# nka77/DAHiTra

Hardware: AMD Instinct MI355X
Metric: image-pairs/s (256x256) train step, 1/2/4/8 MI355X + CPU ref (higher is better)
Workload: dtype bf16; 1 GPU; LEVIR-CD 256x256 synthetic pairs, base_transformer_pos_s4, bf16, batch 32 per GPU (global 32), fwd+focal+bwd+allreduce+AdamW; net_G=base_transformer_pos_s4, global_batch=32, img_size=256, parallelism=dp1, hip_graph=True, step_form=one graph (AdamW inside), attn_dtype=bf16

## Files before the change

### dahitra_amd/csrc/head_fwd.hip

```cpp
#include "common.h"

namespace {

constexpr int HF_KP = 18;
constexpr int HF_SLOTS = 4;

typedef __attribute__((ext_vector_type(4))) unsigned u32x4;
typedef __attribute__((ext_vector_type(8))) _Float16 hf_f16x8;
constexpr int HF_GPW = 5;

template <typename T, bool INBN>
__global__ __launch_bounds__(256) void head_fwd_kernel(const T* __restrict__ x, const float* __restrict__ w_oihw,
                                                       const float* __restrict__ bias, int NC, const float* __restrict__ in_scale,
                                                       const float* __restrict__ in_shift, int in_groups, float* __restrict__ out,
                                                       int N, int H, int W, int rpb) {
    extern __shared__ __attribute__((aligned(16))) float smem[];
    const int RS = (W + 2) * HF_KP;
    const int tid = threadIdx.x, lane = tid & 63, wv = tid >> 6, pl = lane & 15, g = lane >> 4;
    const int bpi = (H + rpb - 1) / rpb, n = blockIdx.x / bpi, r0 = (blockIdx.x - n * bpi) * rpb, r1 = min(r0 + rpb, H);
    constexpr bool F32 = sizeof(T) == 4;
    constexpr int PL = F32 ? 2 : 1, PXB = 32 * (int)sizeof(T);
    uint4 a0[PL], a1[PL];
    {
        float v0[8], v1[8];
        const int tap = pl >> 1, co = pl & 1;
#pragma unroll
        for (int e = 0; e < 8; ++e) {
            const int ci = 8 * g + e;
            v0[e] = co < NC ? w_oihw[((size_t)co * 32 + ci) * 9 + tap] : 0.f;
            v1[e] = (pl < 2 && pl < NC) ? w_oihw[((size_t)pl * 32 + ci) * 9 + 8] : 0.f;
            if constexpr (F32) { v0[e] *= F32H3_WSCALE; v1[e] *= F32H3_WSCALE; }
        }
        if constexpr (F32) { split_f16_planes(v0, a0); split_f16_planes(v1, a1); }
        else { a0[0] = pack16<bf16>(v0); a1[0] = pack16<bf16>(v1); }
    }
    auto mma = [](const uint4& a, const uint4& b, f32x4 c) {
        if constexpr (F32) return __builtin_amdgcn_mfma_f32_16x16x32_f16(__builtin_bit_cast(hf_f16x8, a), __builtin_bit_cast(hf_f16x8, b), c, 0, 0, 0);
        else return __builtin_amdgcn_mfma_f32_16x16x32_bf16(__builtin_bit_cast(s16x8, a), __builtin_bit_cast(s16x8, b), c, 0, 0, 0);
    };
// ... 67 lines not shown
                *reinterpret_cast<float2*>(p + 4 * g + 2) = make_float2(d0[2], d0[3]);
                if (g == 0) *reinterpret_cast<float2*>(p + 16) = make_float2(d1[0], d1[1]);
            }
        }
    };
    const float b0 = bias ? bias[0] : 0.f, b1 = (bias && NC > 1) ? bias[1] : 0.f;
    auto out_row = [&](int y) {
        const float* s0 = smem + ((y - 1) & (HF_SLOTS - 1)) * RS;
        const float* s1 = smem + (y & (HF_SLOTS - 1)) * RS;
        const float* s2 = smem + ((y + 1) & (HF_SLOTS - 1)) * RS;
        for (int xx = tid; xx < W; xx += 256) {
            float acc0 = b0, acc1 = b1;
#pragma unroll
            for (int kh = 0; kh < 3; ++kh) {
                const float* s = kh == 0 ? s0 : (kh == 1 ? s1 : s2);
#pragma unroll
                for (int kw = 0; kw < 3; ++kw) {
                    const float2 v = *reinterpret_cast<const float2*>(s + (xx + kw) * HF_KP + (kh * 3 + kw) * 2);
                    acc0 += v.x; acc1 += v.y;
                }
            }
            out[(((long)n * NC) * H + y) * W + xx] = acc0;
            if (NC > 1) out[(((long)n * NC + 1) * H + y) * W + xx] = acc1;
        }
    };
    RowRegs qa, qb;
    request(r0 - 1, qa);
    request(r0, qb);
    p_row(r0 - 1, qa);
    request(r0 + 1, qa);
    p_row(r0, qb);
    for (int y = r0; y < r1; y += 2) {
        request(y + 2, qb);
        p_row(y + 1, qa);
        __syncthreads();
        out_row(y);
        if (y + 1 >= r1) break;
        request(y + 3, qa);
        p_row(y + 2, qb);
        __syncthreads();
        out_row(y + 1);
    }
}

}

extern "C" int dh_head_fwd_supported(int NC, int W) { return NC >= 1 && NC <= 2 && (long)HF_SLOTS * (W + 2) * HF_KP * 4 <= 80 * 1024; }
extern "C" int dh_head_fwd(int dtype, const void* x, const float* w_oihw, const float* bias, int NC, const float* in_scale,
                           const float* in_shift, int in_groups, float* logits_nchw, int N, int H, int W, void* stream) {
    DH_REQUIRE(x && w_oihw && logits_nchw && N > 0 && H > 0 && W > 0, "head_fwd: bad arguments");
    DH_REQUIRE(dh_head_fwd_supported(NC, W), "head_fwd: n_class=%d W=%d is not this kernel's shape (dh_head_fwd_supported)", NC, W);
    DH_REQUIRE((long)N * H * W * 128 < (1L << 31), "head_fwd: %d x %d x %d pixels x 128 bytes do not fit a 2 GiB buffer descriptor", N, H, W);
    if (in_scale) DH_REQUIRE(in_shift && in_groups > 0 && N % in_groups == 0, "head_fwd: BatchNorm-on-load needs in_shift and N %% in_groups == 0");
    int rpb = H;
    while (rpb > 8 && (long)N * ((H + rpb / 2 - 1) / (rpb / 2)) <= 512) rpb /= 2;
    const int grid = N * ((H + rpb - 1) / rpb);
    const size_t lds = (size_t)HF_SLOTS * (W + 2) * HF_KP * 4;
    hipStream_t st = reinterpret_cast<hipStream_t>(stream);
    static bool attr_done = false;
    if (!attr_done) {
        DH_REQUIRE(hipFuncSetAttribute(reinterpret_cast<const void*>(head_fwd_kernel<bf16, true>), hipFuncAttributeMaxDynamicSharedMemorySize, 80 * 1024) == hipSuccess &&
                   hipFuncSetAttribute(reinterpret_cast<const void*>(head_fwd_kernel<bf16, false>), hipFuncAttributeMaxDynamicSharedMemorySize, 80 * 1024) == hipSuccess &&
                   hipFuncSetAttribute(reinterpret_cast<const void*>(head_fwd_kernel<float, true>), hipFuncAttributeMaxDynamicSharedMemorySize, 80 * 1024) == hipSuccess &&
                   hipFuncSetAttribute(reinterpret_cast<const void*>(head_fwd_kernel<float, false>), hipFuncAttributeMaxDynamicSharedMemorySize, 80 * 1024) == hipSuccess,
                   "head_fwd: 80 KiB of dynamic LDS refused");
        attr_done = true;
    }
#define HF_LAUNCH(T, BN) hipLaunchKernelGGL((head_fwd_kernel<T, BN>), dim3(grid), dim3(256), lds, st, (const T*)x, w_oihw, bias, NC, in_scale, \
                                            in_shift, BN ? in_groups : 1, logits_nchw, N, H, W, rpb)
    if (dtype == DH_DTYPE_BF16) { if (in_scale) HF_LAUNCH(bf16, true); else HF_LAUNCH(bf16, false); }
    else { if (in_scale) HF_LAUNCH(float, true); else HF_LAUNCH(float, false); }
#undef HF_LAUNCH
    DH_CHECK_LAUNCH("head_fwd");
    return 0;
}
```

### dahitra_amd/csrc/loss_optim.hip

```cpp
#include "common.h"

namespace {

constexpr int MAXC = 8;

template <int CT>
__global__ __launch_bounds__(256) void focal_kernel(const float* __restrict__ logits, const long long* __restrict__ target,
                                                    int B, int Crt, long HW, float alpha, float gscale,
                                                    float* __restrict__ dlogits, float* __restrict__ partial) {
    __shared__ float red[256];
    const int C = CT > 0 ? CT : Crt;
    constexpr int NC = CT > 0 ? CT : MAXC;
    const long total = (long)B * HW;
    float lsum = 0.f;
    const long stride = (long)gridDim.x * blockDim.x;
    const long i0 = (long)blockIdx.x * blockDim.x + threadIdx.x;
    long b = i0 / HW, p = i0 - b * HW;
    const long db = stride / HW, dp = stride - db * HW;
    for (long i = i0; i < total; i += stride) {
        float z[NC], pr[NC], lp[NC];
        float m = -INFINITY;
#pragma unroll
        for (int c = 0; c < NC; ++c)
            if (c < C) { z[c] = logits[(b * C + c) * HW + p]; m = fmaxf(m, z[c]); }
        float s = 0.f;
#pragma unroll
        for (int c = 0; c < NC; ++c)
            if (c < C) { pr[c] = expf(z[c] - m); s += pr[c]; }
        const float ls = logf(s), inv = 1.f / s;
        const int t = (int)target[i];
        float loss = 0.f, gsum = 0.f, gp[NC];
#pragma unroll
        for (int c = 0; c < NC; ++c)
            if (c < C) {
                pr[c] *= inv;
                lp[c] = z[c] - m - ls;
                const float oh = (c == t ? 1.f : 0.f) + 1e-6f;
                const float om = 1.f - pr[c];
                loss += oh * (-alpha * om * om * lp[c]);
                gp[c] = oh * (-alpha) * (-2.f * om * pr[c] * lp[c] + om * om);
                gsum += gp[c];
            }
        lsum += loss;
        if (dlogits) {
#pragma unroll
            for (int c = 0; c < NC; ++c)
                if (c < C) dlogits[(b * C + c) * HW + p] = gscale * (gp[c] - pr[c] * gsum);
        }
        b += db; p += dp;
        if (p >= HW) { p -= HW; ++b; }
    }
    red[threadIdx.x] = lsum;
    __syncthreads();
    for (int o = 128; o > 0; o >>= 1) {
        if (threadIdx.x < o) red[threadIdx.x] += red[threadIdx.x + o];
        __syncthreads();
    }
    if (threadIdx.x == 0) partial[blockIdx.x] = red[0];
}

__global__ __launch_bounds__(256) void ce_partial_kernel(const float* __restrict__ logits, const long long* __restrict__ target,
                                                         int B, int C, long HW, int ignore, double* __restrict__ partial) {
    __shared__ double sh[16];
    double ls = 0.0, cnt = 0.0;
    const long total = (long)B * HW;
    for (long i = (long)blockIdx.x * blockDim.x + threadIdx.x; i < total; i += (long)gridDim.x * blockDim.x) {
        const int t = (int)target[i];
        if (t == ignore) continue;
        const long b = i / HW, p = i % HW;
        float m = -INFINITY;
// ... 352 lines not shown
```

### dahitra_amd/engine.py

```python
import os
import sys
import types

import torch

from . import ops
from .netspec import (ATTN_SCALE, BIT_DIM_HEAD, BIT_HEADS, BN_EPS, BN_MOMENTUM, DIM, LN_EPS, UNET_LEVELS,
                      get_config, is_active, state_spec)

RELU, GELU, NONE = ops.ACT_RELU, ops.ACT_GELU, ops.ACT_NONE



def _drain(gen):
    try:
        while True:
            next(gen)
    except StopIteration as e:
        return e.value


class Packed:
    __slots__ = ("fwd", "dgrad", "fwd_frag", "dgrad_frag")

    def __init__(self, fwd, dgrad, fwd_frag=None, dgrad_frag=None):
        self.fwd, self.dgrad, self.fwd_frag, self.dgrad_frag = fwd, dgrad, fwd_frag, dgrad_frag


class Gated:
    __slots__ = ("g", "partial")

    def __init__(self, g, partial):
        self.g, self.partial = g, partial


class HeadGrad:
    __slots__ = ("dl", "w", "ncls", "gw", "gb")

    def __init__(self, dl, w, ncls, gw, gb):
        self.dl, self.w, self.ncls, self.gw, self.gb = dl, w, ncls, gw, gb


class CoarseRes:
    __slots__ = ("t",)

    def __init__(self, t):
        self.t = t


class MaskedRes:
    __slots__ = ("t", "bits")

    def __init__(self, t, bits):
        self.t, self.bits = t, bits


class Engine:
    def __init__(self, net_G, dtype=torch.float32, use_tr=True, attn_fp8=False, mma_x3=False):
        self.net_G = net_G
        self.mma_x3 = bool(mma_x3) and dtype == torch.float32
        self.mma_fwd = int(os.environ.get("DAHITRA_X3_FWD", "3")) if self.mma_x3 else 0
        self.mma_bwd = int(os.environ.get("DAHITRA_X3_BWD", "1")) if self.mma_x3 else 0
        self._x3_checked = False
        self.attn_fp8 = bool(attn_fp8) or os.environ.get("DAHITRA_ATTN_FP8", "0") == "1"
        self.cfg = get_config(net_G)
        self.dtype = dtype
        self.use_tr = use_tr
        self.fused_decoder = os.environ.get("DAHITRA_NO_FUSED_DECODER", "0") != "1"
        self.fused_encoder = os.environ.get("DAHITRA_NO_FUSED_ENCODER", "0") != "1"
        self.fused_bn_bwd = os.environ.get("DAHITRA_BN_FUSION", "0") == "1"
        self.coarse_shortcut = os.environ.get("DAHITRA_NO_COARSE_SHORTCUT", "0") != "1"
        self.lazy_bn = os.environ.get("DAHITRA_NO_LAZY_BN", "0") != "1"
        self.phase_conv_pred = os.environ.get("DAHITRA_NO_PHASE_CONV", "0") != "1"
        self.phase_s2_dgrad = os.environ.get("DAHITRA_NO_PHASE_S2", "0") != "1"
        self.phase_up_conv = os.environ.get("DAHITRA_NO_PHASE_UPCONV", "0") != "1"
        self.split_cat = os.environ.get("DAHITRA_NO_SPLIT_CAT", "0") != "1"
        self.direct_stem = os.environ.get("DAHITRA_NO_DIRECT_STEM", "0") != "1"
        self.fused_stem_bwd = os.environ.get("DAHITRA_NO_FUSED_STEM_BWD", "0") != "1"
        self.fused_head_out = os.environ.get("DAHITRA_NO_FUSED_HEAD", "0") != "1"
        self.defer_dec_finalize = os.environ.get("DAHITRA_NO_DEFER_DEC_FINALIZE", "0") != "1"
        self.fuse_dec_stack = os.environ.get("DAHITRA_NO_DEC_STACK", "0") != "1"
        self.level_streams = os.environ.get("DAHITRA_LEVEL_STREAMS", "0") == "1"
        self._lstreams = []
        self.gated_head_dgrad = os.environ.get("DAHITRA_GATED_HEAD", "0") == "1"
        self.fused_head_bn = os.environ.get("DAHITRA_NO_FUSED_HEAD_BN", "0") != "1"
        self.fused_up4_bwd = os.environ.get("DAHITRA_NO_FUSED_UP4_BWD", "0") != "1"
        self.fused_up4_fwd = os.environ.get("DAHITRA_FUSED_UP4_FWD", "0") == "1"
        self.use_side = os.environ.get("DAHITRA_SIDE_STREAM", "0") == "1"
        self.block_copies = os.environ.get("DAHITRA_BLOCK_COPIES", "0") == "1"
        self.pack_side = os.environ.get("DAHITRA_PACK_SIDE", "0") == "1"
        self._pack_stream = None
        self.side = None
        self._deferred_wgrad = None
        self.shapes = {k: s for k, s, _ in state_spec(net_G)}
        self.p = {}
        self.g = {}
        self.pk = {}
        self.wstack = {}
        self.training = False
        self.need_grad = False
        self._bwd = None
        self._plans = {}
        self._wgrad_plan = None

    def bind(self, params, grads):
        self.p, self.g = params, grads
        self._plans = {}

# ... 753 lines not shown
    def run_deferred_wgrad(self):
        d, self._deferred_wgrad = self._deferred_wgrad, None
        if d is None:
            return
        x, dy, wkey, ks, stride, pad, dilation = d
        with self.side.fork(x.y if isinstance(x, ops.BnInput) else (x.a if isinstance(x, ops.Up4Input) else x), dy):
            ops.conv2d_wgrad(x, dy, self.g[wkey], ks, stride, pad, accumulate=True, use_tr=self.use_tr, dilation=dilation)

    def _side_join(self):
        if self.side is not None:
            self.run_deferred_wgrad()
            self.side.join()

    def backward_second(self):
        ops.set_f32_mma_mode(self.mma_bwd)
        second, state = self._split_state
        self._split_state = None
        try:
            second(state)
            self._wgrad_plan.run()
        finally:
            self._wgrad_plan.__exit__(*sys.exc_info())

    def _head_out(self, h, wkey, bkey):
        ncls = self.shapes[wkey][0]
        ck = ops.chunk_channels(self.dtype)
        if self.pk[wkey].fwd.shape[-2] == 16 and self.fused_head_out:
            out = ops.conv3x3_head(h, self.pk[wkey].fwd, ncls, self.p[bkey], w_oihw=self.p[wkey])
        else:
            out = ops.nhwc_to_nchw(ops.conv2d(h, self.pk[wkey].fwd, ncls, 3, 1, 1, bias=self.p[bkey]))
        if not self.need_grad:
            return out, None

        small = 8 if (self.dtype == torch.bfloat16 or ncls > 4) else 4
        direct = h.shape[-1] == 32 and ncls <= small

        def bwd(dl_nchw, next_gate=None, head_bn=None, relu_out=None):
            if direct and next_gate is None:
                fuse = self.fused_head_bn and ncls <= 8 and self.g[wkey].is_contiguous() and \
                    (self.dtype == torch.bfloat16 or (self.dtype == torch.float32 and ops.get_f32_mma_mode() != 0))
                if head_bn is not None and fuse:
                    return HeadGrad(ops.head_dlogits_pack(dl_nchw, self.dtype), self.p[wkey], ncls, self.g[wkey], self.g[bkey])
                if relu_out is not None and fuse and relu_out is h:
                    return ops.head_relu_bwd(ops.head_dlogits_pack(dl_nchw, self.dtype), self.p[wkey], ncls, h, self.g[wkey],
                                             self.g[bkey])
                dl = ops.nchw_to_nhwc(dl_nchw, self.dtype, cpad=small)
                ops.conv2d_wgrad(h, dl, self.g[wkey], 3, 1, 1, accumulate=True, use_tr=self.use_tr, cout_real=ncls)
                tmp = torch.empty(small, dtype=torch.float32, device=h.device)
                ops.colsum(dl.view(-1, small), tmp)
                ops.reduce_rows(tmp, 1, ncls, self.g[bkey], accumulate=True)
                if head_bn is not None and self.gated_head_dgrad and self.dtype == torch.bfloat16 and ncls <= 2:
                    return Gated(*ops.head_dgrad3x3_bn(dl, self.p[wkey], ncls, *head_bn))
                return ops.head_dgrad3x3(dl, self.p[wkey], ncls, relu_out=relu_out)
            dl = ops.nchw_to_nhwc(dl_nchw, self.dtype, cpad=ck)
            ops.conv2d_wgrad(h, dl, self.g[wkey], 3, 1, 1, accumulate=True, use_tr=self.use_tr, cout_real=ncls)
            tmp = torch.empty(ck, dtype=torch.float32, device=h.device)
            ops.colsum(dl.view(-1, ck), tmp)
            ops.reduce_rows(tmp, 1, ncls, self.g[bkey], accumulate=True)
            dh = self.conv_dgrad(dl, wkey, 3, 1, 1, h.shape, gate=next_gate)
            return ops.act_bwd(dh, relu_out, RELU) if relu_out is not None else dh
# ... 16 lines not shown
        phased = self.phase_conv_pred and l3.shape[-1] % 64 == 0
        if phased:
            feat, b_pred = self.conv_pred_phase(l3)
        else:
            up = ops.upsample2(l3)
            feat, b_pred = self.conv_act(up, "conv_pred.weight", "conv_pred.bias", 3, 1, NONE)
        _, fh, fw, _ = feat.shape
        hw = fh * fw
        wa = self.p["conv_a.weight"]
        tok_cat, tsaved = ops.tokenizer_fwd(feat, wa, self.p["pos_embedding"], B, L)
        tok2d, b_enc = self.encoder(tok_cat.view(B * 2 * L, DIM), "transformer", cfg["enc_depth"], BIT_HEADS,
                                    BIT_DIM_HEAD, B, 2 * L)
        dtok = torch.zeros_like(tok2d) if self.need_grad else None
        dec, b_dec = self.decoder(feat.view(S2 * hw, DIM), S2, tok2d, 2 * L * DIM, L * DIM, B, dtok,
                                  "transformer_decoder", cfg["dec_depth"], BIT_HEADS, cfg["dec_dim_head"], L)
        dec4 = dec.view(S2, fh, fw, DIM)
        k0 = "classifier.0.weight"
        if self.fused_up4_fwd and self.dtype == torch.bfloat16 and DIM == 32 and tuple(self.shapes[k0][:2]) == (32, 32) and \
                tuple(self.pk[k0].fwd.shape) == (9, 32, 32):
            upd = ops.Up4Input(dec4[:B].contiguous(), dec4[B:].contiguous())
        else:
            upd = ops.absdiff_upsample4(dec4[:B], dec4[B:])
        h, b_c0 = self.conv_bn(upd, k0, "classifier.1", 3, 1, 1, 1, True, lazy=True, side_wgrad=True)
        logits, b_out = self._head_out(h, "classifier.3.weight", "classifier.3.bias")
        if not self.need_grad:
            return logits, None

        def bwd_first(dl):
            dh = b_out(dl, next_gate=b_c0.gate, head_bn=getattr(b_c0, "bn", None))
            fuse = self.fused_up4_bwd and self.dtype == torch.bfloat16 and fh % 2 == 0 and fw % 4 == 0 and \
                self.pk["classifier.0.weight"].dgrad.dim() == 3 and self.pk["classifier.0.weight"].dgrad.shape[1] == 32
            if fuse:
                dec_g = torch.empty_like(dec4)
                b_c0(dh, through_up4=(dec4[:B], dec4[B:], dec_g[:B], dec_g[B:]))
            else:
                dupd, _ = b_c0(dh)
                dec_g = torch.empty_like(dec4)
                ops.absdiff_upsample4_bwd_into(dec4[:B], dec4[B:], dupd, dec_g[:B], dec_g[B:])
            dfeat = b_dec(dec_g.view(S2 * hw, DIM))
            if self.side is not None:
                self.run_deferred_wgrad()
            dtok_cat = b_enc(dtok)
            dfeat4 = dfeat.view(S2, fh, fw, DIM)
            ops.tokenizer_bwd(feat, wa, tsaved, dtok_cat, dfeat4, self.g["conv_a.weight"], self.g["pos_embedding"],
                              B, L, accumulate=True)
            dl3 = b_pred(dfeat4) if phased else ops.upsample2_bwd(b_pred(dfeat4))
            return b_l3(dl3, next_gate=b_l2.gate)
# ... 167 lines not shown
        s4, b_l1 = self.res_layer(p4, 1, 1, 2)
        s8, b_l2 = self.res_layer(s4, 2, 2, 2)
        p16, arg16 = ops.maxpool(s8, want_arg=True)
        s16, b_l3 = self.res_layer(p16, 3, 1, 2)
        level = self._xbd_level if self.cfg["kind"] == "xbd" else self._level
        if self.need_grad:
            self._zpool = [torch.zeros(3 * 3 * B * self.cfg["token_len"] * DIM, dtype=torch.float32, device=s4.device), 0]
        ew = self.cfg["kind"] != "xbd"
        (o5, b5), (t4, b4), (t3, b3) = self._run_staged([level(5, s16, B), level(4, s8, B), level(3, s4, B)], ew=ew)
        self._zpool = None
        o5u = ops.upsample2(o5)
        o4, bu4 = self._up_conv(4, ops.add(t4, o5u))
        o3, bu3 = self._up_conv(3, ops.add(t3, o4))
        _, h2, w2, c2 = s2.shape
        k20 = "conv_layer2_0.0.weight"
        split2 = self.split_cat and self.training and self.pk[k20].fwd_frag is not None and \
            (not self.need_grad or self.pk[k20].dgrad_frag is not None) and \
            ops.conv3x3_split_supported(B, h2, w2, 2 * c2, self.shapes[k20][0], self.dtype)
        cat2 = ops.SplitCat(s2) if split2 else ops.SplitCat(s2).materialize()
        y, b20 = self.conv_bn(cat2, k20, "conv_layer2_0.1", 3, 1, 1, 1, True, lazy=True)
        y2 = ops.conv2d(y, self.pk["conv_layer2_0.3.weight"].fwd, 32, 3, 1, 1, bias=self.p["conv_layer2_0.3.bias"],
                        residual=o3)
        o2, bu2 = self._up_conv(2, y2)
        logits, b_out = self._head_out(o2, "classifier.weight", "classifier.bias")
        if not self.need_grad:
            return logits, None

        def bwd_first(dl):
            do2 = b_out(dl, relu_out=o2)
            dy2 = bu2(do2, masked=True)
            ops.conv2d_wgrad(y, dy2, self.g["conv_layer2_0.3.weight"], 3, 1, 1, accumulate=True, use_tr=self.use_tr)
            ops.colsum(dy2.view(-1, 32), self.g["conv_layer2_0.3.bias"], accumulate=True)
            dy = self.conv_dgrad(dy2, "conv_layer2_0.3.weight", 3, 1, 1, y.shape, gate=b20.gate)
            dcat2, _ = b20(dy)
            if split2:
                ds2 = dcat2
            else:
                ds2 = ops.split_halves(dcat2)
            dsum3 = bu3(dy2)
            dsum4 = bu4(dsum3)
            ds4, ds8, ds16 = self._run_staged([b3(dsum3), b4(dsum4), b5(ops.upsample2_bwd(dsum4))], ew=ew)
            return ds16, ds8, ds4, ds2

        def bwd_second(state):
            ds16, ds8, ds4, ds2 = state
            dp16 = b_l3(ds16)
            ds8 = ops.add(ds8, ops.maxpool_bwd(arg16, dp16, s8.shape))
# ... 12 lines not shown
```

### dahitra_amd/graph.py

```python
import os

import torch
import torch.distributed as dist

from . import ops, parallel
from .models import losses


class GraphedTrainStep:
    CHECK_EVERY = 64

    def __init__(self, net, opt, a, b, lab, warmup=3, confusion=None):
        if not getattr(opt, "capturable", False):
            raise ValueError("GraphedTrainStep needs dahitra_amd.optim.AdamW(..., capturable=True)")
        self.net, self.opt = net, opt
        self.confusion = confusion
        self.world = dist.get_world_size() if dist.is_initialized() else 1
        self.exchange = parallel.exchange_enabled()
        self.split_off = None
        self.persist_bn_launches = None
        self._set_inputs(a, b, lab)
        net._ensure_arena(a.device)
        flat0 = net._arena.flat.clone()
        bufs0 = [t.clone() for t in net.buffers()]
# ... 59 lines not shown
        loss.backward()
        self._count(self.logits)
        if include_opt:
            self.opt.step()
        return loss.detach()

    def _body(self, include_opt):
        if type(self)._eager_body is not GraphedTrainStep._eager_body or os.environ.get("DAHITRA_GRAPH_AUTOGRAD") == "1":
            return self._eager_body(include_opt)
        net = self.net
        logits = self._forward_split()
        bwd = net._engine.take_backward()
        self.logits = logits
        loss, dl = self._loss_and_grad(logits)
        self._count(logits)
        net._arena.grad.zero_()
        net._engine.backward(dl, bwd)
        net._bind_grad_views()
        if include_opt:
            self.opt.step()
        return loss

    def _forward_split(self):
        return self.net._run_forward(self.a, self.b, need_grad=True)

    def _loss_and_grad(self, logits):
        tgt = self.lab[:, 0] if self.lab.dim() == logits.dim() else self.lab
        return ops.focal_loss(logits, tgt.to(torch.int64).contiguous(), want_grad=True)

    def _count(self, logits):
        if self.confusion is not None:
            tgt = self.lab[:, 0] if self.lab.dim() == logits.dim() else self.lab
            ops.confusion_matrix(logits, tgt.to(torch.int64).contiguous(), self.confusion)

    def _can_split(self):
        self.split_off = parallel.split_offset(self.net, self.world)
        return self.split_off is not None

    def _split_first(self):
        net = self.net
        logits = self._forward_split()
        bwd = net._engine.take_backward()
        self.logits = logits
        loss, dl = self._loss_and_grad(logits)
        self._count(logits)
        net._arena.grad.zero_()
        net._engine.backward_first(dl, bwd)
        net._bind_grad_views()
        return loss
# ... 451 lines not shown
```

### dahitra_amd/ops.py

```python
import bisect
import ctypes
import math
import os
import sys

import numpy as np
import torch

from . import _lib

ACT_NONE, ACT_RELU, ACT_GELU = 0, 1, 2
_DT = {torch.float32: 0, torch.bfloat16: 1}
_vp = ctypes.c_void_p


def dt(t):
    try:
        return _DT[t.dtype]
    except KeyError:
        raise TypeError("dahitra_amd: unsupported activation dtype %s" % t.dtype)


def set_f32_mma_mode(mode):
    _lib.check(_lib.lib().dh_set_f32_mma_mode(int(mode)), "dh_set_f32_mma_mode")
# ... 492 lines not shown

HEAD_FWD = os.environ.get("DAHITRA_NO_HEAD_FWD", "0") != "1"


def conv3x3_head(x, wp, ncls, bias, w_oihw=None):
    bn_in = x if isinstance(x, BnInput) else None
    if bn_in is not None:
        x = bn_in.y
    N, H, W, Cin = x.shape
    assert wp.shape[-2] == 16 and ncls <= 16
    out = torch.empty(N, ncls, H, W, dtype=torch.float32, device=x.device)
    if HEAD_FWD and w_oihw is not None and Cin == 32 and N * H * W * 128 < 2 ** 31 and _lib.lib().dh_head_fwd_supported(ncls, W) and \
            (x.dtype == torch.bfloat16 or (x.dtype == torch.float32 and get_f32_mma_mode() == 3)):
        assert w_oihw.shape == (ncls, 32, 3, 3) and w_oihw.dtype == torch.float32
        with _Prof("head_fwd", 2.0 * N * H * W * ncls * Cin * 9, _nb(x, out)):
            _call("dh_head_fwd", dt(x), P(x), P(w_oihw), P(bias), ncls, *_bn_in_args(bn_in), P(out), N, H, W, S())
        return out
    key = "conv_mfma<%s,ks3,s1,nt16>" % ("bf16" if x.dtype == torch.bfloat16 else "f32")
    with _Prof(key, 2.0 * N * H * W * ncls * Cin * 9, _nb(x, out, wp)):
        _call("dh_conv3x3_head_fwd", dt(x), P(x), P(wp), P(bias), N, H, W, Cin, ncls, *_bn_in_args(bn_in), P(out), S())
    return out


def rows_view(x2d):
    rows, C = x2d.shape
    return rows, cdiv(rows, 16), C


def linear(x2d, wp, cout, bias=None, residual=None, act=ACT_NONE, want_preact=False, images=1, w_image_stride=0):
    rows, Cin = x2d.shape
    rpi = rows // images
    Hh = cdiv(rpi, 16)
    cpad = wp.shape[-2]
    y = torch.empty(rows, cout, dtype=x2d.dtype, device=x2d.device)
    pre = torch.empty_like(y) if want_preact else None
    _call("dh_conv2d_fwd", dt(x2d), P(x2d), P(wp), P(y), P(bias), P(residual), _vp(0), images, Hh, 16, Cin, Hh, 16, cout, cpad, 1,
          1, 0, act, rpi, w_image_stride, P(pre), 1, *_gate_args(None), *_bn_in_args(None), 0, _vp(0), S())
    assert images == 1 or rpi % 16 == 0
    return (y, pre) if want_preact else y


def conv2d_wgrad(x, dy, dw, ks, stride, pad, accumulate=False, groups=1, use_tr=True, cout_real=0, cin=0, dilation=1,
                 defer=True):
    if isinstance(x, BnInput):
        return _conv2d_wgrad_bn_in(x, dy, dw, ks, stride, pad, accumulate, use_tr, cout_real, dilation, defer)
    if isinstance(x, SplitCat):
# ... 1525 lines not shown
```

### include/dahitra_hip.h

```cpp
#ifndef DAHITRA_HIP_H
#define DAHITRA_HIP_H
#ifdef __cplusplus
extern "C" {
#endif

#define DH_F32 0
#define DH_BF16 1
#define DH_ACT_NONE 0
#define DH_ACT_RELU 1
#define DH_ACT_GELU 2

int dh_abi_version(void);
const char* dh_last_error(void);
void dh_set_error(const char* msg);

int dh_conv2d_fwd(int dtype, const void* x, const void* w_packed, void* y, const float* bias,
                  const void* residual, float* stats_partial, int N, int H, int W, int Cin, int OH, int OW,
                  int Cout, int CoutPad, int ks, int stride, int pad, int act, int npix_valid,
                  long w_image_stride, void* y_preact, int dilation, const void* gate_out, const void* gate_y,
                  const float* gate_mean, const float* gate_invstd, int gate_groups, const float* in_scale,
                  const float* in_shift, int in_groups, int phase_mode, const void* w_frag, void* stream);
int dh_conv2d_fwd_num_tiles(int dtype, int N, int OH, int OW, int Cin, int ks, int stride);
int dh_conv2d_fwd_describe(int entry, int dtype, int N, int H, int W, int Cin, int OH, int OW, int Cout, int CoutPad, int ks, int stride,
                           int pad, int act, int npix_valid, long w_image_stride, int dilation, int gate_groups, int in_groups,
// ... 132 lines not shown
                             const unsigned char* post_label, const int* idx, const int* params, const int* coef,
                             const int* jitter_host, int N, int H, int W, int S, int mode, float* out_img, unsigned char* out_msk,
                             unsigned char* out_lbl, void* workspace, long workspace_bytes, void* stream);
int dh_nchw_to_nhwc(int dtype, const float* src, void* dst, int N, int C, long HW, int CP, void* stream);
int dh_head_dgrad3x3(int dtype, const void* dy, int CP, const float* w_oihw, int NC, void* dx, int N, int H, int W,
                     void* stream);
int dh_head_dgrad3x3_relu(const void* dy, const float* w_oihw, int NC, const void* relu_out, void* dx, int N, int H, int W,
                          void* stream);
int dh_head_dgrad3x3_bn_blocks(int N, int H, int W, int groups);
int dh_head_dgrad3x3_bn(const void* dy, const float* w_oihw, int NC, const void* y, const float* mask_scale, const float* mask_shift,
                        const float* mean, const float* invstd, int groups, void* g, float* partial, int N, int H, int W,
                        void* stream);
int dh_head_bn_bwd_blocks(int N, int H, int W, int groups);
long dh_head_bn_bwd_workspace_size(int N, int H, int W, int groups);
int dh_head_dlogits_pack(int dtype, const float* dlogits_nchw, int N, int NC, int H, int W, void* dlp, void* stream);
int dh_head_bn_bwd(int dtype, const void* dlp, const float* w_oihw, int NC, const void* y, const float* mask_scale, const float* mask_shift,
                   const float* mean, const float* invstd, const float* gamma, int groups, void* dx, float* dgamma, float* dbeta,
                   float* dw, float* db, int accumulate, int N, int H, int W, void* workspace, void* stream);
int dh_head_relu_bwd(int dtype, const void* dlp, const float* w_oihw, int NC, const void* relu_out, void* dx, float* dw, float* db,
                     int accumulate, int N, int H, int W, void* workspace, void* stream);
int dh_head_fwd_supported(int NC, int W);
int dh_head_fwd(int dtype, const void* x, const float* w_oihw, const float* bias, int NC, const float* in_scale, const float* in_shift,
                int in_groups, float* logits_nchw, int N, int H, int W, void* stream);
enum { DH_EW_ADD_POS = 1, DH_EW_CAT_HALVES = 2, DH_EW_SPLIT_HALVES = 3, DH_EW_ABSDIFF_HALVES = 4, DH_EW_ABSDIFF_HALVES_BWD = 5,
       DH_EW_ADD_POS_BWD = 6 };
int dh_ew_multi(int n, const int* op, const void* const* a, const void* const* b, void* const* c, const int* i0, const int* i1,
                const long* l0, void* stream);
int dh_nhwc_to_nchw(int dtype, const void* src, float* dst, int N, int C, long HW, void* stream);
int dh_copy_channels(int dtype, const void* src, int Cs, int sc0, void* dst, int Cd, int dc0, int Cn, long P, void* stream);
int dh_cat_halves(int dtype, void* t, void* cat, int C, long P, int inverse, void* stream);
int dh_add(int dtype, const void* a, const void* b, void* y, long n, void* stream);
int dh_add_pos(int dtype, const void* x, const float* pos, void* y, int N, long HW, int C, void* stream);
int dh_add_pos_bwd(int dtype, const void* dy, float* dpos, int N, long HW, int C, int accumulate, void* stream);
int dh_act_bwd(int dtype, const void* dy, const void* ref, void* dx, long n, int act, void* stream);
int dh_maxpool3x3s2_fwd(int dtype, const void* x, void* y, unsigned char* argmax, int N, int H, int W, int C,
                        const float* bn_scale, const float* bn_shift, int groups, void* stream);
int dh_maxpool3x3s2_bwd(int dtype, const unsigned char* argmax, const void* dy, void* dx, int N, int H, int W, int C, void* stream);
int dh_upsample2_nearest_fwd(int dtype, const void* x, void* y, int N, int H, int W, int C, void* stream);
int dh_upsample2_nearest_bwd(int dtype, const void* dy, void* dx, int N, int H, int W, int C, void* stream);
int dh_absdiff_upsample4_fwd(int dtype, const void* a, const void* b, void* y, int N, int H, int W, int C, void* stream);
int dh_absdiff_upsample4_bwd(int dtype, const void* a, const void* b, const void* dy, void* da, void* db, int N, int H, int W, int C, void* stream);
int dh_absdiff(int dtype, const void* a, const void* b, void* y, long n, void* stream);
int dh_absdiff_bwd(int dtype, const void* a, const void* b, const void* dy, void* da, void* db, long n, int accumulate, void* stream);
int dh_colsum(int dtype, const void* x, long P, int C, float* out, int accumulate, void* workspace, void* stream);
int dh_cast_from_f32(int dtype, const float* src, void* dst, long n, void* stream);
int dh_cast_to_f32(int dtype, const void* src, float* dst, long n, int accumulate, void* stream);
// ... 173 lines not shown
```

Baseline: 10170 image-pairs/s.

## Fuse focal loss and packed dlogits into the head conv forward kernel

Adds a head_fwd_loss kernel that computes the focal loss per pixel and its gradient right after the 3x3 head convolution. The gradient is written directly as packed bf16 pairs in the padded layout the head backward consumes, and the training graph uses this fused result instead of a separate focal-loss pass. This removes a re-read of the fp32 logits, a separate dlogits write and the later pack kernel. In exchange it adds a per-pixel loss-terms buffer with a small reduction, and the head backward must now accept packed dlogits.

```diff
diff --git a/dahitra_amd/csrc/focal_pixel.h b/dahitra_amd/csrc/focal_pixel.h
--- /dev/null
+++ b/dahitra_amd/csrc/focal_pixel.h
@@ -0,0 +1,35 @@
+#pragma once
+#include <hip/hip_runtime.h>
+
+template <int NC>
+__device__ __forceinline__ float dh_focal_pixel(const float (&z)[NC], int C, int t, float alpha, float gscale, float (&dl)[NC]) {
+#pragma clang fp contract(off)
+    float d[NC], e[NC], pr[NC], gp[NC];
+    float m = -INFINITY;
+#pragma unroll
+    for (int c = 0; c < NC; ++c)
+        if (c < C) m = fmaxf(m, z[c]);
+    float s = 0.f;
+#pragma unroll
+    for (int c = 0; c < NC; ++c)
+        if (c < C) { d[c] = z[c] - m; e[c] = expf(d[c]); s += e[c]; }
+    const float ls = logf(s), inv = 1.f / s;
+    float loss = 0.f, gsum = 0.f;
+#pragma unroll
+    for (int c = 0; c < NC; ++c)
+        if (c < C) {
+            pr[c] = e[c] * inv;
+            const float lp = d[c] - ls;
+            const float oh = (c == t ? 1.f : 0.f) + 1e-6f;
+            const float om = fmaf(-inv, e[c], 1.f);
+            loss += oh * (-alpha * om * om * lp);
+            const float inner = fmaf(-2.f * om * pr[c], lp, om * om);
+            const float a = oh * (-alpha);
+            gp[c] = a * inner;
+            gsum = fmaf(a, inner, gsum);
+        }
+#pragma unroll
+    for (int c = 0; c < NC; ++c)
+        if (c < C) dl[c] = gscale * fmaf(-pr[c], gsum, gp[c]);
+    return loss;
+}
diff --git a/dahitra_amd/csrc/head_fwd.hip b/dahitra_amd/csrc/head_fwd.hip
--- a/dahitra_amd/csrc/head_fwd.hip
+++ b/dahitra_amd/csrc/head_fwd.hip
@@ -1,20 +1,24 @@
 #include "common.h"
+#include "focal_pixel.h"
+#include "head_fwd_plan.h"
 
 namespace {
-
-constexpr int HF_KP = 18;
-constexpr int HF_SLOTS = 4;
 
 typedef __attribute__((ext_vector_type(4))) unsigned u32x4;
 typedef __attribute__((ext_vector_type(8))) _Float16 hf_f16x8;
-constexpr int HF_GPW = 5;
-
-template <typename T, bool INBN>
-__global__ __launch_bounds__(256) void head_fwd_kernel(const T* __restrict__ x, const float* __restrict__ w_oihw,
-                                                       const float* __restrict__ bias, int NC, const float* __restrict__ in_scale,
-                                                       const float* __restrict__ in_shift, int in_groups, float* __restrict__ out,
-                                                       int N, int H, int W, int rpb) {
-    extern __shared__ __attribute__((aligned(16))) float smem[];
+
+struct HeadLossArgs {
+    const long long* target;
+    unsigned* dlp;
+    float* terms;
+    float alpha, gscale;
+};
+
+template <typename T, bool INBN, bool LOSS>
+__device__ __forceinline__ void head_fwd_body(float* smem, const T* __restrict__ x, const float* __restrict__ w_oihw,
+                                              const float* __restrict__ bias, int NC, const float* __restrict__ in_scale,
+                                              const float* __restrict__ in_shift, int in_groups, float* __restrict__ out,
+                                              int N, int H, int W, int rpb, const HeadLossArgs& la) {
     const int RS = (W + 2) * HF_KP;
     const int tid = threadIdx.x, lane = tid & 63, wv = tid >> 6, pl = lane & 15, g = lane >> 4;
     const int bpi = (H + rpb - 1) / rpb, n = blockIdx.x / bpi, r0 = (blockIdx.x - n * bpi) * rpb, r1 = min(r0 + rpb, H);
@@ -128,6 +132,13 @@
             }
             out[(((long)n * NC) * H + y) * W + xx] = acc0;
             if (NC > 1) out[(((long)n * NC + 1) * H + y) * W + xx] = acc1;
+            if constexpr (LOSS) {
+                const float z[2] = {acc0, acc1};
+                float dl[2];
+                const long px = ((long)n * H + y) * W + xx;
+                la.terms[px] = dh_focal_pixel<2>(z, 2, (int)la.target[px], la.alpha, la.gscale, dl);
+                la.dlp[hf_dlp_index(n, y, xx, H, W)] = f2bf2(dl[0], dl[1]);
+            }
         }
     };
     RowRegs qa, qb;
@@ -149,29 +160,69 @@
     }
 }
 
-}
-
-extern "C" int dh_head_fwd_supported(int NC, int W) { return NC >= 1 && NC <= 2 && (long)HF_SLOTS * (W + 2) * HF_KP * 4 <= 80 * 1024; }
+template <typename T, bool INBN>
+__global__ __launch_bounds__(256) void head_fwd_kernel(const T* __restrict__ x, const float* __restrict__ w_oihw,
+                                                       const float* __restrict__ bias, int NC, const float* __restrict__ in_scale,
+                                                       const float* __restrict__ in_shift, int in_groups, float* __restrict__ out,
+                                                       int N, int H, int W, int rpb) {
+    extern __shared__ __attribute__((aligned(16))) float smem[];
+    head_fwd_body<T, INBN, false>(smem, x, w_oihw, bias, NC, in_scale, in_shift, in_groups, out, N, H, W, rpb, HeadLossArgs{});
+}
+
+template <bool INBN>
+__global__ __launch_bounds__(256) void head_fwd_loss_kernel(const bf16* __restrict__ x, const float* __restrict__ w_oihw,
+                                                            const float* __restrict__ bias, const float* __restrict__ in_scale,
+                                                            const float* __restrict__ in_shift, int in_groups, float* __restrict__ out,
+                                                            int N, int H, int W, int rpb, HeadLossArgs la) {
+    extern __shared__ __attribute__((aligned(16))) float smem[];
+    head_fwd_body<bf16, INBN, true>(smem, x, w_oihw, bias, 2, in_scale, in_shift, in_groups, out, N, H, W, rpb, la);
+}
+
+__global__ __launch_bounds__(256) void focal_terms_sum_kernel(const float* __restrict__ terms, long total, float* __restrict__ partial) {
+    __shared__ float red[256];
+    float lsum = 0.f;
+    const long stride = (long)gridDim.x * blockDim.x;
+    for (long i = (long)blockIdx.x * blockDim.x + threadIdx.x; i < total; i += stride) lsum += terms[i];
+    red[threadIdx.x] = lsum;
+    __syncthreads();
+    for (int o = 128; o > 0; o >>= 1) {
+        if (threadIdx.x < o) red[threadIdx.x] += red[threadIdx.x + o];
+        __syncthreads();
+    }
+    if (threadIdx.x == 0) partial[blockIdx.x] = red[0];
+}
+
+}
+
+extern "C" int dh_reduce_partials(const float* partial, long nt, long n, float scale, float* out, int accumulate, void* stream);
+extern "C" int dh_head_fwd_supported(int NC, int W) { return hf_shape_ok(NC, W); }
+
+static int head_fwd_lds_attr() {
+    static bool attr_done = false;
+    if (!attr_done) {
+        DH_REQUIRE(hipFuncSetAttribute(reinterpret_cast<const void*>(head_fwd_kernel<bf16, true>), hipFuncAttributeMaxDynamicSharedMemorySize, 80 * 1024) == hipSuccess &&
+                   hipFuncSetAttribute(reinterpret_cast<const void*>(head_fwd_kernel<bf16, false>), hipFuncAttributeMaxDynamicSharedMemorySize, 80 * 1024) == hipSuccess &&
+                   hipFuncSetAttribute(reinterpret_cast<const void*>(head_fwd_kernel<float, true>), hipFuncAttributeMaxDynamicSharedMemorySize, 80 * 1024) == hipSuccess &&
+                   hipFuncSetAttribute(reinterpret_cast<const void*>(head_fwd_kernel<float, false>), hipFuncAttributeMaxDynamicSharedMemorySize, 80 * 1024) == hipSuccess &&
+                   hipFuncSetAttribute(reinterpret_cast<const void*>(head_fwd_loss_kernel<true>), hipFuncAttributeMaxDynamicSharedMemorySize, 80 * 1024) == hipSuccess &&
+                   hipFuncSetAttribute(reinterpret_cast<const void*>(head_fwd_loss_kernel<false>), hipFuncAttributeMaxDynamicSharedMemorySize, 80 * 1024) == hipSuccess,
+                   "head_fwd: 80 KiB of dynamic LDS refused");
+        attr_done = true;
+    }
+    return 0;
+}
+
 extern "C" int dh_head_fwd(int dtype, const void* x, const float* w_oihw, const float* bias, int NC, const float* in_scale,
                            const float* in_shift, int in_groups, float* logits_nchw, int N, int H, int W, void* stream) {
     DH_REQUIRE(x && w_oihw && logits_nchw && N > 0 && H > 0 && W > 0, "head_fwd: bad arguments");
     DH_REQUIRE(dh_head_fwd_supported(NC, W), "head_fwd: n_class=%d W=%d is not this kernel's shape (dh_head_fwd_supported)", NC, W);
     DH_REQUIRE((long)N * H * W * 128 < (1L << 31), "head_fwd: %d x %d x %d pixels x 128 bytes do not fit a 2 GiB buffer descriptor", N, H, W);
     if (in_scale) DH_REQUIRE(in_shift && in_groups > 0 && N % in_groups == 0, "head_fwd: BatchNorm-on-load needs in_shift and N %% in_groups == 0");
-    int rpb = H;
-    while (rpb > 8 && (long)N * ((H + rpb / 2 - 1) / (rpb / 2)) <= 512) rpb /= 2;
-    const int grid = N * ((H + rpb - 1) / rpb);
-    const size_t lds = (size_t)HF_SLOTS * (W + 2) * HF_KP * 4;
+    const HeadFwdPlan pl = hf_plan(NC, N, H, W);
+    const int grid = pl.grid, rpb = pl.rpb;
+    const size_t lds = pl.lds;
     hipStream_t st = reinterpret_cast<hipStream_t>(stream);
-    static bool attr_done = false;
-    if (!attr_done) {
-        DH_REQUIRE(hipFuncSetAttribute(reinterpret_cast<const void*>(head_fwd_kernel<bf16, true>), hipFuncAttributeMaxDynamicSharedMemorySize, 80 * 1024) == hipSuccess &&
-                   hipFuncSetAttribute(reinterpret_cast<const void*>(head_fwd_kernel<bf16, false>), hipFuncAttributeMaxDynamicSharedMemorySize, 80 * 1024) == hipSuccess &&
-                   hipFuncSetAttribute(reinterpret_cast<const void*>(head_fwd_kernel<float, true>), hipFuncAttributeMaxDynamicSharedMemorySize, 80 * 1024) == hipSuccess &&
-                   hipFuncSetAttribute(reinterpret_cast<const void*>(head_fwd_kernel<float, false>), hipFuncAttributeMaxDynamicSharedMemorySize, 80 * 1024) == hipSuccess,
-                   "head_fwd: 80 KiB of dynamic LDS refused");
-        attr_done = true;
-    }
+    if (int e = head_fwd_lds_attr()) return e;
 #define HF_LAUNCH(T, BN) hipLaunchKernelGGL((head_fwd_kernel<T, BN>), dim3(grid), dim3(256), lds, st, (const T*)x, w_oihw, bias, NC, in_scale, \
                                             in_shift, BN ? in_groups : 1, logits_nchw, N, H, W, rpb)
     if (dtype == DH_DTYPE_BF16) { if (in_scale) HF_LAUNCH(bf16, true); else HF_LAUNCH(bf16, false); }
@@ -180,3 +231,35 @@
     DH_CHECK_LAUNCH("head_fwd");
     return 0;
 }
+
+extern "C" int dh_head_fwd_loss_supported(int dtype, int NC, int H, int W, int groups) { return hf_loss_ok(dtype, NC, H, W, groups); }
+extern "C" int dh_head_fwd_loss_workspace_size(int N, int H, int W) {
+    return hf_plan(2, N, H, W).ok ? (int)hf_loss_workspace_bytes(N, H, W) : 0;
+}
+extern "C" int dh_head_fwd_loss(int dtype, const void* x, const float* w_oihw, const float* bias, int NC, const float* in_scale,
+                                const float* in_shift, int in_groups, const long long* target, float alpha, float grad_scale,
+                                float* logits_nchw, void* dlp, float* loss_out, int N, int H, int W, void* workspace, void* stream) {
+    DH_REQUIRE(x && w_oihw && logits_nchw && target && dlp && loss_out && workspace && N > 0 && H > 0 && W > 0, "head_fwd_loss: bad arguments");
+    DH_REQUIRE(dh_head_fwd_loss_supported(dtype, NC, H, W, in_scale ? in_groups : 0),
+               "head_fwd_loss: dtype=%d n_class=%d W=%d is not this kernel's shape (dh_head_fwd_loss_supported)", dtype, NC, W);
+    if (in_scale) DH_REQUIRE(in_shift && in_groups > 0 && N % in_groups == 0, "head_fwd_loss: BatchNorm-on-load needs in_shift and N %% in_groups == 0");
+    const HeadFwdPlan pl = hf_plan(NC, N, H, W);
+    DH_REQUIRE(pl.ok, "head_fwd_loss: %d x %d x %d pixels x 128 bytes do not fit a 2 GiB buffer descriptor", N, H, W);
+    hipStream_t st = reinterpret_cast<hipStream_t>(stream);
+    if (int e = head_fwd_lds_attr()) return e;
+    const long total = (long)N * H * W;
+    float* partial = reinterpret_cast<float*>(workspace);
+    float* terms = partial + HF_SUM_BLOCKS_MAX;
+    const HeadLossArgs la = {target, reinterpret_cast<unsigned*>(dlp), terms, alpha, grad_scale / (float)total};
+    if (in_scale)
+        hipLaunchKernelGGL((head_fwd_loss_kernel<true>), dim3(pl.grid), dim3(256), pl.lds, st, (const bf16*)x, w_oihw, bias, in_scale, in_shift,
+                           in_groups, logits_nchw, N, H, W, pl.rpb, la);
+    else
+        hipLaunchKernelGGL((head_fwd_loss_kernel<false>), dim3(pl.grid), dim3(256), pl.lds, st, (const bf16*)x, w_oihw, bias, in_scale, in_shift,
+                           1, logits_nchw, N, H, W, pl.rpb, la);
+    DH_CHECK_LAUNCH("head_fwd_loss");
+    const int g = hf_sum_blocks(total);
+    hipLaunchKernelGGL(focal_terms_sum_kernel, dim3(g), dim3(256), 0, st, terms, total, partial);
+    DH_CHECK_LAUNCH("focal_terms_sum");
+    return dh_reduce_partials(partial, g, 1, 1.0f / (float)total, loss_out, 0, stream);
+}
diff --git a/dahitra_amd/csrc/head_fwd_plan.h b/dahitra_amd/csrc/head_fwd_plan.h
--- /dev/null
+++ b/dahitra_amd/csrc/head_fwd_plan.h
@@ -0,0 +1,47 @@
+#pragma once
+#include <stddef.h>
+
+#ifndef DH_DTYPE_F32
+#define DH_DTYPE_F32 0
+#define DH_DTYPE_BF16 1
+#endif
+
+constexpr int HF_KP = 18;
+constexpr int HF_SLOTS = 4;
+constexpr int HF_GPW = 5;
+constexpr long HF_LDS_MAX = 80 * 1024;
+
+struct HeadFwdPlan {
+    int ok;
+    int rpb;
+    int grid;
+    size_t lds;
+};
+
+inline int hf_shape_ok(int NC, int W) { return NC >= 1 && NC <= 2 && W > 0 && (long)HF_SLOTS * (W + 2) * HF_KP * 4 <= HF_LDS_MAX; }
+
+inline HeadFwdPlan hf_plan(int NC, int N, int H, int W) {
+    HeadFwdPlan p = {0, 0, 0, 0};
+    if (!hf_shape_ok(NC, W) || N <= 0 || H <= 0 || (long)N * H * W * 128 >= (1L << 31)) return p;
+    int rpb = H;
+    while (rpb > 8 && (long)N * ((H + rpb / 2 - 1) / (rpb / 2)) <= 512) rpb /= 2;
+    p.ok = 1;
+    p.rpb = rpb;
+    p.grid = N * ((H + rpb - 1) / rpb);
+    p.lds = (size_t)HF_SLOTS * (W + 2) * HF_KP * 4;
+    return p;
+}
+
+inline int hf_loss_ok(int dtype, int NC, int H, int W, int groups) {
+    return dtype == DH_DTYPE_BF16 && NC == 2 && H > 0 && groups >= 0 && hf_shape_ok(NC, W);
+}
+inline long hf_dlp_words(int N, int H, int W) { return (long)N * (H + 2) * (W + 2); }
+constexpr long hf_dlp_index(int n, int y, int x, int H, int W) { return ((long)n * (H + 2) + y + 1) * (W + 2) + x + 1; }
+constexpr int HF_SUM_BLOCKS_MAX = 1024;
+inline int hf_sum_blocks(long total) {
+    const long g = (total + 255) / 256;
+    return (int)(g > HF_SUM_BLOCKS_MAX ? HF_SUM_BLOCKS_MAX : g);
+}
+inline long hf_loss_workspace_bytes(int N, int H, int W) {
+    return (N > 0 && H > 0 && W > 0) ? ((long)HF_SUM_BLOCKS_MAX + (long)N * H * W) * 4 : 0;
+}
diff --git a/dahitra_amd/csrc/loss_optim.hip b/dahitra_amd/csrc/loss_optim.hip
--- a/dahitra_amd/csrc/loss_optim.hip
+++ b/dahitra_amd/csrc/loss_optim.hip
@@ -1,4 +1,5 @@
 #include "common.h"
+#include "focal_pixel.h"
 
 namespace {
 
@@ -18,34 +19,45 @@
     long b = i0 / HW, p = i0 - b * HW;
     const long db = stride / HW, dp = stride - db * HW;
     for (long i = i0; i < total; i += stride) {
-        float z[NC], pr[NC], lp[NC];
-        float m = -INFINITY;
-#pragma unroll
-        for (int c = 0; c < NC; ++c)
-            if (c < C) { z[c] = logits[(b * C + c) * HW + p]; m = fmaxf(m, z[c]); }
-        float s = 0.f;
-#pragma unroll
-        for (int c = 0; c < NC; ++c)
-            if (c < C) { pr[c] = expf(z[c] - m); s += pr[c]; }
-        const float ls = logf(s), inv = 1.f / s;
-        const int t = (int)target[i];
-        float loss = 0.f, gsum = 0.f, gp[NC];
-#pragma unroll
-        for (int c = 0; c < NC; ++c)
-            if (c < C) {
-                pr[c] *= inv;
-                lp[c] = z[c] - m - ls;
-                const float oh = (c == t ? 1.f : 0.f) + 1e-6f;
-                const float om = 1.f - pr[c];
-                loss += oh * (-alpha * om * om * lp[c]);
-                gp[c] = oh * (-alpha) * (-2.f * om * pr[c] * lp[c] + om * om);
-                gsum += gp[c];
+        if constexpr (CT == 2) {
+            float z[2], dl[2];
+            z[0] = logits[(b * 2) * HW + p];
+            z[1] = logits[(b * 2 + 1) * HW + p];
+            lsum += dh_focal_pixel<2>(z, 2, (int)target[i], alpha, gscale, dl);
+            if (dlogits) {
+                dlogits[(b * 2) * HW + p] = dl[0];
+                dlogits[(b * 2 + 1) * HW + p] = dl[1];
             }
-        lsum += loss;
-        if (dlogits) {
+        } else {
+            float z[NC], pr[NC], lp[NC];
+            float m = -INFINITY;
 #pragma unroll
             for (int c = 0; c < NC; ++c)
-                if (c < C) dlogits[(b * C + c) * HW + p] = gscale * (gp[c] - pr[c] * gsum);
+                if (c < C) { z[c] = logits[(b * C + c) * HW + p]; m = fmaxf(m, z[c]); }
+            float s = 0.f;
+#pragma unroll
+            for (int c = 0; c < NC; ++c)
+                if (c < C) { pr[c] = expf(z[c] - m); s += pr[c]; }
+            const float ls = logf(s), inv = 1.f / s;
+            const int t = (int)target[i];
+            float loss = 0.f, gsum = 0.f, gp[NC];
+#pragma unroll
+            for (int c = 0; c < NC; ++c)
+                if (c < C) {
+                    pr[c] *= inv;
+                    lp[c] = z[c] - m - ls;
+                    const float oh = (c == t ? 1.f : 0.f) + 1e-6f;
+                    const float om = 1.f - pr[c];
+                    loss += oh * (-alpha * om * om * lp[c]);
+                    gp[c] = oh * (-alpha) * (-2.f * om * pr[c] * lp[c] + om * om);
+                    gsum += gp[c];
+                }
+            lsum += loss;
+            if (dlogits) {
+#pragma unroll
+                for (int c = 0; c < NC; ++c)
+                    if (c < C) dlogits[(b * C + c) * HW + p] = gscale * (gp[c] - pr[c] * gsum);
+            }
         }
         b += db; p += dp;
         if (p >= HW) { p -= HW; ++b; }
diff --git a/dahitra_amd/engine.py b/dahitra_amd/engine.py
--- a/dahitra_amd/engine.py
+++ b/dahitra_amd/engine.py
@@ -39,6 +39,17 @@
 
     def __init__(self, dl, w, ncls, gw, gb):
         self.dl, self.w, self.ncls, self.gw, self.gb = dl, w, ncls, gw, gb
+
+
+class PackedDlogits:
+    __slots__ = ("dlp",)
+
+    def __init__(self, dlp):
+        self.dlp = dlp
+
+    @property
+    def device(self):
+        return self.dlp.device
 
 
 class CoarseRes:
@@ -84,6 +95,10 @@
         self._lstreams = []
         self.gated_head_dgrad = os.environ.get("DAHITRA_GATED_HEAD", "0") == "1"
         self.fused_head_bn = os.environ.get("DAHITRA_NO_FUSED_HEAD_BN", "0") != "1"
+        self.fused_head_loss = os.environ.get("DAHITRA_NO_FUSED_HEAD_LOSS", "0") != "1"
+        self.loss_target = None
+        self.head_loss = None
+        self._dlp_bufs = {}
         self.fused_up4_bwd = os.environ.get("DAHITRA_NO_FUSED_UP4_BWD", "0") != "1"
         self.fused_up4_fwd = os.environ.get("DAHITRA_FUSED_UP4_FWD", "0") == "1"
         self.use_side = os.environ.get("DAHITRA_SIDE_STREAM", "0") == "1"
@@ -883,10 +898,22 @@
         finally:
             self._wgrad_plan.__exit__(*sys.exc_info())
 
-    def _head_out(self, h, wkey, bkey):
+    def _head_out(self, h, wkey, bkey, packed_bwd=False):
         ncls = self.shapes[wkey][0]
         ck = ops.chunk_channels(self.dtype)
-        if self.pk[wkey].fwd.shape[-2] == 16 and self.fused_head_out:
+        tgt, self.loss_target, self.head_loss = self.loss_target, None, None
+        y = h.y if isinstance(h, ops.BnInput) else h
+        if tgt is not None and packed_bwd and self.need_grad and self.fused_head_loss and self.fused_head_out and \
+                self.fused_head_bn and not self.gated_head_dgrad and self.dtype == torch.bfloat16 and ncls == 2 and \
+                ops.PROFILE is None and self.pk[wkey].fwd.shape[-2] == 16 and self.g[wkey].is_contiguous() and \
+                tuple(tgt.shape) == tuple(y.shape[:3]) and ops.head_fwd_loss_supported(h, ncls):
+            key = (tuple(y.shape[:3]), str(y.device))
+            dlp = self._dlp_bufs.get(key)
+            if dlp is None:
+                dlp = self._dlp_bufs[key] = ops.head_dlp_buffer(*y.shape[:3], y.device)
+            out, loss = ops.head_fwd_loss(h, self.p[wkey], self.p[bkey], tgt, dlp)
+            self.head_loss = (loss, PackedDlogits(dlp))
+        elif self.pk[wkey].fwd.shape[-2] == 16 and self.fused_head_out:
             out = ops.conv3x3_head(h, self.pk[wkey].fwd, ncls, self.p[bkey], w_oihw=self.p[wkey])
         else:
             out = ops.nhwc_to_nchw(ops.conv2d(h, self.pk[wkey].fwd, ncls, 3, 1, 1, bias=self.p[bkey]))
@@ -897,6 +924,13 @@
         direct = h.shape[-1] == 32 and ncls <= small
 
         def bwd(dl_nchw, next_gate=None, head_bn=None, relu_out=None):
+            if isinstance(dl_nchw, PackedDlogits):
+                fuse = direct and next_gate is None and self.fused_head_bn and self.g[wkey].is_contiguous()
+                if fuse and head_bn is not None:
+                    return HeadGrad(dl_nchw.dlp, self.p[wkey], ncls, self.g[wkey], self.g[bkey])
+                if fuse and relu_out is not None and relu_out is h:
+                    return ops.head_relu_bwd(dl_nchw.dlp, self.p[wkey], ncls, h, self.g[wkey], self.g[bkey])
+                raise RuntimeError("dahitra_amd: packed dlogits reached a head backward that cannot take them")
             if direct and next_gate is None:
                 fuse = self.fused_head_bn and ncls <= 8 and self.g[wkey].is_contiguous() and \
                     (self.dtype == torch.bfloat16 or (self.dtype == torch.float32 and ops.get_f32_mma_mode() != 0))
@@ -959,7 +993,8 @@
         else:
             upd = ops.absdiff_upsample4(dec4[:B], dec4[B:])
         h, b_c0 = self.conv_bn(upd, k0, "classifier.1", 3, 1, 1, 1, True, lazy=True, side_wgrad=True)
-        logits, b_out = self._head_out(h, "classifier.3.weight", "classifier.3.bias")
+        logits, b_out = self._head_out(h, "classifier.3.weight", "classifier.3.bias",
+                                       packed_bwd=b_c0 is not None and b_c0.gate is None and getattr(b_c0, "bn", None) is not None)
         if not self.need_grad:
             return logits, None
 
@@ -1173,7 +1208,7 @@
         y2 = ops.conv2d(y, self.pk["conv_layer2_0.3.weight"].fwd, 32, 3, 1, 1, bias=self.p["conv_layer2_0.3.bias"],
                         residual=o3)
         o2, bu2 = self._up_conv(2, y2)
-        logits, b_out = self._head_out(o2, "classifier.weight", "classifier.bias")
+        logits, b_out = self._head_out(o2, "classifier.weight", "classifier.bias", packed_bwd=True)
         if not self.need_grad:
             return logits, None
 
diff --git a/dahitra_amd/graph.py b/dahitra_amd/graph.py
--- a/dahitra_amd/graph.py
+++ b/dahitra_amd/graph.py
@@ -105,9 +105,18 @@
         return loss
 
     def _forward_split(self):
-        return self.net._run_forward(self.a, self.b, need_grad=True)
+        eng = self.net._engine
+        tgt = self.lab[:, 0] if self.lab.dim() == 4 else self.lab
+        eng.head_loss, eng.loss_target = None, tgt.to(torch.int64).contiguous()
+        try:
+            return self.net._run_forward(self.a, self.b, need_grad=True)
+        finally:
+            eng.loss_target = None
 
     def _loss_and_grad(self, logits):
+        fused, self.net._engine.head_loss = self.net._engine.head_loss, None
+        if fused is not None:
+            return fused
         tgt = self.lab[:, 0] if self.lab.dim() == logits.dim() else self.lab
         return ops.focal_loss(logits, tgt.to(torch.int64).contiguous(), want_grad=True)
 
diff --git a/dahitra_amd/ops.py b/dahitra_amd/ops.py
--- a/dahitra_amd/ops.py
+++ b/dahitra_amd/ops.py
@@ -538,6 +538,40 @@
     return out
 
 
+HEAD_LOSS_LAUNCHES = 0
+
+
+def head_fwd_loss_supported(x, ncls):
+    bn_in = x if isinstance(x, BnInput) else None
+    y = bn_in.y if bn_in is not None else x
+    N, H, W, Cin = y.shape
+    return bool(HEAD_FWD and Cin == 32 and N * H * W * 128 < 2 ** 31 and y.dtype in _DT and
+                _lib.lib().dh_head_fwd_loss_supported(_DT[y.dtype], ncls, H, W, bn_in.groups if bn_in is not None else 0))
+
+
+def head_dlp_buffer(N, H, W, device):
+    return torch.zeros(_head_dlp_shape(N, H, W, 2, torch.bfloat16), dtype=torch.int32, device=device)
+
+
+def head_fwd_loss(x, w_oihw, bias, target, dlp, grad_scale=1.0, alpha=0.5):
+    global HEAD_LOSS_LAUNCHES
+    bn_in = x if isinstance(x, BnInput) else None
+    if bn_in is not None:
+        x = bn_in.y
+    N, H, W, _ = x.shape
+    assert w_oihw.shape == (2, 32, 3, 3) and w_oihw.dtype == torch.float32 and x.is_contiguous()
+    assert target.dtype == torch.int64 and tuple(target.shape) == (N, H, W) and target.is_contiguous()
+    assert dlp.dtype == torch.int32 and tuple(dlp.shape) == (N, H + 2, W + 2) and dlp.is_contiguous()
+    out = torch.empty(N, 2, H, W, dtype=torch.float32, device=x.device)
+    loss = torch.empty((), dtype=torch.float32, device=x.device)
+    ws = workspace(_lib.lib().dh_head_fwd_loss_workspace_size(N, H, W), x.device)
+    with _Prof("head_fwd_loss", 2.0 * N * H * W * 2 * 32 * 9, _nb(x, out, target, dlp)):
+        _call("dh_head_fwd_loss", dt(x), P(x), P(w_oihw), P(bias), 2, *_bn_in_args(bn_in), P(target), alpha, grad_scale, P(out),
+              P(dlp), P(loss), N, H, W, P(ws), S())
+    HEAD_LOSS_LAUNCHES += 1
+    return out, loss
+
+
 def rows_view(x2d):
     rows, C = x2d.shape
     return rows, cdiv(rows, 16), C
diff --git a/include/dahitra_hip.h b/include/dahitra_hip.h
--- a/include/dahitra_hip.h
+++ b/include/dahitra_hip.h
@@ -178,6 +178,11 @@
 int dh_head_fwd_supported(int NC, int W);
 int dh_head_fwd(int dtype, const void* x, const float* w_oihw, const float* bias, int NC, const float* in_scale, const float* in_shift,
                 int in_groups, float* logits_nchw, int N, int H, int W, void* stream);
+int dh_head_fwd_loss_supported(int dtype, int NC, int H, int W, int groups);
+int dh_head_fwd_loss_workspace_size(int N, int H, int W);
+int dh_head_fwd_loss(int dtype, const void* x, const float* w_oihw, const float* bias, int NC, const float* in_scale,
+                     const float* in_shift, int in_groups, const long long* target, float alpha, float grad_scale,
+                     float* logits_nchw, void* dlp, float* loss_out, int N, int H, int W, void* workspace, void* stream);
 enum { DH_EW_ADD_POS = 1, DH_EW_CAT_HALVES = 2, DH_EW_SPLIT_HALVES = 3, DH_EW_ABSDIFF_HALVES = 4, DH_EW_ABSDIFF_HALVES_BWD = 5,
        DH_EW_ADD_POS_BWD = 6 };
 int dh_ew_multi(int n, const int* op, const void* const* a, const void* const* b, void* const* c, const int* i0, const int* i1,
```

Result: no change. 10220 image-pairs/s (median of 6 runs) (+0.5%).
